# HydrogenSulfate/LFT

Measured on AMD Instinct MI355X. Metric: LF patches/sec (5x5 angRes, 32x32 LR, 4xSR), higher is better.
Workload: dtype bf16; 1 GPU; LFT 5x5 angRes 4xSR inference, batch=4 per GPU, 32x32 LR patches; global_batch=4, parallelism=dp1 (independent shards), streams_per_gpu=1, hip_graph=True, steps_in_flight=2

## Files before the change

### lft_amd/csrc/lft_api.hip

```cpp
#include "../../include/lft_hip.h"
#include "../../include/lft_hip_test.h"
#include <hip/hip_runtime.h>
#include <stdint.h>

#include <cstdarg>
#include <cstdio>
#include <cmath>
#include <map>
#include <mutex>
#include <set>
#include <string>
#include <algorithm>
#include <type_traits>
#include <utility>
#include <vector>

#ifndef LFT_TU
#define LFT_TU 0
#endif

namespace {
#include "lft_kernels_a.cuh"
#include "lft_kernels_b.cuh"
#include "lft_metrics.cuh"
// ... 92 lines not shown
    return fail(LFT_ERR_ARG, "internal: no kernel variant for %d", (int)v);
}
template <int V> using int_c = std::integral_constant<int, V>;
template <typename F> int by_prec(int prec, F&& f) {
    if (prec == LFT_PREC_F32) return f(float{});
    if (prec == LFT_PREC_BF16) return f(bf16_t{});
    return f(f16_t{});
}
inline size_t align256(size_t x) { return (x + 255) & ~(size_t)255; }

struct Dims {
    int B, A, V, h, w, hw, s, gp, gt, nchunk;
    long long ntok;
};

int make_dims(int B, int A, int h, int w, int s, int prec, Dims* d) {
    if (prec != LFT_PREC_F32 && prec != LFT_PREC_BF16 && prec != LFT_PREC_F16)
        return fail(LFT_ERR_ARG, "prec must be LFT_PREC_F32, LFT_PREC_BF16 or LFT_PREC_F16, got %d", prec);
    if (B < 1 || A < 1 || h < 1 || w < 1) return fail(LFT_ERR_SHAPE, "B, A, h, w must be positive (B=%d A=%d h=%d w=%d)", B, A, h, w);
    if (s != 2 && s != 4) return fail(LFT_ERR_SHAPE, "scale factor must be 2 or 4, got %d", s);
    if (A * A > 128) return fail(LFT_ERR_UNSUPPORTED, "angRes %d (A*A=%d views > 128) is not implemented in this build", A, A * A);
    if ((long long)B * A * A * h * w > (1LL << 27)) return fail(LFT_ERR_SHAPE, "too many tokens");
    d->B = B; d->A = A; d->V = A * A; d->h = h; d->w = w; d->hw = h * w; d->s = s;
    d->gp = (s + 2) * (s + 2); d->gt = (d->gp + 31) / 32; d->nchunk = 2 * s * s;
    d->ntok = (long long)B * d->V * d->hw;
    return 0;
}

constexpr int kFragsConv = 72, kFragsAng = 64, kFragsSpa1 = 240, kFragsSpa1NoQ = 208, kFragsSpa2 = 176;
inline int frags_up(const Dims& d) { return d.nchunk * (4 + 2 * d.gt); }

struct PackedLayout {
    size_t conv0_w, ln_ang[kLayers], ln_spa[kLayers], ang_pe, petok[kLayers], spa_pe_img;
    size_t w01, s_w01;
    size_t s_conv[3], s_ang[kLayers], s_spa1[kLayers], s_spa2[kLayers], s_up, total;
};

PackedLayout packed_layout(const Dims& d, int prec) {
    const size_t esz = prec == LFT_PREC_F32 ? 4 : 2, fragb = 64 * 8 * esz;
    PackedLayout L;
    size_t o = 0;
    auto take = [&](size_t bytes) { size_t r = o; o = align256(o + bytes); return r; };
    L.conv0_w = take(576 * 4);
    for (int l = 0; l < kLayers; ++l) { L.ln_ang[l] = take(256 * 4); L.ln_spa[l] = take(512 * 4); }
    L.ang_pe = take((size_t)((d.V + 31) / 32) * 2048 * 4);
    for (int l = 0; l < kLayers; ++l) L.petok[l] = take((size_t)((d.hw + 32 * kNwSpa1 - 1) / (32 * kNwSpa1)) * kNwSpa1 * 4096 * esz);
    L.spa_pe_img = take((size_t)d.hw * 64 * esz);
    const bool lp = prec != LFT_PREC_F32;
    L.w01 = take(lp ? 64 * kW01K * 4 : 0);
    L.s_conv[0] = take(kFragsConv * fragb);
    L.s_w01 = take(lp ? kW01Frags * fragb : 0);
    for (int i = 1; i < 3; ++i) L.s_conv[i] = take(kFragsConv * fragb);
    for (int l = 0; l < kLayers; ++l) {
        L.s_ang[l] = take(kFragsAng * fragb);
        L.s_spa1[l] = take(kFragsSpa1 * fragb);
        L.s_spa2[l] = take(kFragsSpa2 * fragb);
    }
    L.s_up = take((size_t)frags_up(d) * fragb);
    L.total = o;
    return L;
}

struct WorkLayout {
    size_t x0, feat, xa, xb, tok, q, k, v, o, g, status, total;
};
WorkLayout work_layout(const Dims& d, int prec) {
    const size_t esz = prec == LFT_PREC_F32 ? 4 : 2;
    WorkLayout W;
    size_t o = 0;
    auto take = [&](size_t bytes) { size_t r = o; o = align256(o + bytes); return r; };
    const size_t n = (size_t)d.ntok;
    W.x0 = take(n * 64 * esz); W.feat = take(n * 64 * esz); W.xa = take(n * 64 * esz); W.xb = take(n * 64 * esz);
    W.tok = take(n * 128 * esz); W.q = take(n * 128 * esz); W.k = take(n * 128 * esz); W.v = take(n * 128 * esz);
    W.o = take(n * 128 * esz);
    W.g = take(n * d.gp * 4);
    W.status = take(256);
    W.total = o;
    return W;
}

template <typename T> size_t lds_conv64(int w) { return WRing<T, kConv64Chunk, kNwConv>::LDS_BYTES + ConvIn<T, kNwConv>::bytes(w) + kNwConv * TileIO<2, T>::BYTES + kConvZeroRow; }
template <typename T> size_t lds_conv64_lr(int w) { return lds_conv64<T>(w) + std::max<size_t>(LrStage<kNwConv>::bytes(w), kConv0WBytes); }
constexpr size_t kLdsParams = 1024;
template <typename T, int CH = kSpaChunk> size_t lds_spa1(int w) {
    return WRing<T, CH, kNwSpa1>::LDS_BYTES + std::max<size_t>(ConvIn<T, kNwSpa1>::bytes(w), (size_t)kNwSpa1 * TileIO<4, T>::BYTES) + kLdsParams + kConvZeroRow;
}
template <typename T> size_t lds_spa2() { return WRing<T, kSpaChunk, kNwSpa2>::LDS_BYTES + kLdsParams + kNwSpa2 * TileIO<4, T>::BYTES; }
template <typename T> size_t lds_up() { return WRing<T, kUpChunk, kNwUp>::LDS_BYTES + kNwUp * TileIO<2, T>::BYTES; }
template <typename T> size_t lds_ang() { return (size_t)kFragsAng * 1024 * FragInfo<T>::PIECES + kLdsParams + 4 * TileIO<2, T>::BYTES; }
constexpr size_t kMaxLds = 160 * 1024;
template <typename K> int allow_lds(K kernel, size_t bytes, const char* name) {
    if (bytes > kMaxLds) return fail(LFT_ERR_SHAPE, "%s needs %zu B of LDS (> 160 KiB): view width too large for this build", name, bytes);
    if (bytes <= 64 * 1024) return 0;
    struct Done { int dev; const void* fn; size_t bytes; };
    static thread_local std::vector<Done> done;
    const void* fn = reinterpret_cast<const void*>(kernel);
    int dev = 0;
    LFT_HIP_OK(hipGetDevice(&dev));
    for (const auto& d : done)
        if (d.dev == dev && d.fn == fn && d.bytes >= bytes) return 0;
    LFT_HIP_OK(hipFuncSetAttribute(fn, hipFuncAttributeMaxDynamicSharedMemorySize, (int)bytes));
    done.push_back(Done{dev, fn, bytes});
    return 0;
}

template <typename P> P* at(const void* base, size_t off) { return reinterpret_cast<P*>(const_cast<char*>(static_cast<const char*>(base)) + off); }
inline unsigned blocks_for(long long items, int per_block) { return (unsigned)((items + per_block - 1) / per_block); }

PackOp lin_op(const float* src, int row0, int nrows, int ld, int k0, int ksteps, int kmap, float scale, int kmul = 1, int kadd = 0) {
    PackOp p{};
    p.src = src; p.kind = 0; p.row0 = row0; p.nrows = nrows; p.ntiles = (nrows + 31) / 32; p.ld = ld;
    p.kmul = kmul; p.kadd = kadd; p.k0 = k0; p.ksteps = ksteps; p.kmap = kmap; p.scale = scale; p.s = 0; p.frag0 = 0;
    return p;
}
void conv_ops(std::vector<PackOp>& v, const float* w, int nout) {
    for (int tap = 0; tap < 9; ++tap)
        for (int ks = 0; ks < 4; ++ks) v.push_back(lin_op(w, 0, nout, 576, 16 * ks, 1, 0, 1.0f, 9, tap));
}

template <typename T>
int run_pack(std::vector<PackOp>& ops, T* dst, int expect_frags, hipStream_t st) {
    int total = 0;
    size_t i = 0;
    while (i < ops.size()) {
        PackArgs a{};
        int nf = 0;
        while (i < ops.size() && a.nops < LFT_PACK_MAXOPS) {
            a.op[a.nops] = ops[i];
            a.op[a.nops].frag0 = nf;
            nf += ops[i].ntiles * ops[i].ksteps;
            ++a.nops; ++i;
        }
        k_pack<T><<<nf, 64, 0, st>>>(a, dst + (size_t)total * 512);
        LFT_LAUNCH_OK("k_pack");
        total += nf;
    }
    if (total != expect_frags) return fail(LFT_ERR_ARG, "internal: stream has %d fragments, expected %d", total, expect_frags);
    return 0;
}

template <typename T> bool tok_lane_major(const Dims& d) {
    return d.hw % (32 * kNwSpa1) == 0 && (sizeof(T) == 4 || d.w % 32 == 0);
}
template <typename T, bool PE_ONLY>
int launch_spa1(unsigned nwg, const T* in, const T* ws, const float* ln, const T* petok, T* tok, T* q, T* k, T* v, T* pe_out,
                int nimg, const Dims& d, hipStream_t st, unsigned* status) {
    const size_t l16 = lds_spa1<T, 16>(d.w), l8 = lds_spa1<T, 8>(d.w);
    const size_t share = kMaxLds / kSpaOcc;
    const bool use8 = (l16 > share && l8 <= share) || l16 > kMaxLds;
    const bool lm = !PE_ONLY && tok_lane_major<T>(d);
    return dispatch<8, 16>(use8 ? 8 : 16, [&](auto CH) {
        return dispatch<true, false>(lm, [&](auto LM) {
            constexpr bool WQ = !(LM && sizeof(T) == 2);
            const size_t lds = CH == 8 ? l8 : l16;
            if (int rc = allow_lds(k_spa1<T, PE_ONLY, CH, LM, WQ>, lds, "k_spa1")) return rc;
            k_spa1<T, PE_ONLY, CH, LM, WQ><<<nwg, 64 * kNwSpa1, lds, st>>>(in, ws, ln, petok, tok, q, k, v, pe_out, nimg, d.h, d.w, status);
            return 0;
        });
    });
}

template <typename T>
int pack_impl(const float* const* P, void* packed, const Dims& d, int prec, hipStream_t st) {
    const PackedLayout L = packed_layout(d, prec);
    const float kAngScale = 0.35355339059327373f * LFT_LOG2E;
    const float kSpaScale = 0.25f * LFT_LOG2E;
    int rc;
    k_copy_f32<<<3, 256, 0, st>>>(P[0], at<float>(packed, L.conv0_w), 576);
    LFT_LAUNCH_OK("k_copy_f32");
    for (int i = 0; i < 3; ++i) {
        std::vector<PackOp> ops;
        conv_ops(ops, P[1 + i], 64);
        if ((rc = run_pack<T>(ops, at<T>(packed, L.s_conv[i]), kFragsConv, st))) return rc;
    }
    if constexpr (sizeof(T) == 2) {
        k_compose_w01<<<blocks_for(64 * kW01K, 256), 256, 0, st>>>(P[0], P[1], at<float>(packed, L.w01));
        LFT_LAUNCH_OK("k_compose_w01");
        std::vector<PackOp> ops{lin_op(at<float>(packed, L.w01), 0, 64, kW01K, 0, kW01K / 16, 0, 1.0f)};
        if ((rc = run_pack<ConvLrOp>(ops, at<ConvLrOp>(packed, L.s_w01), kW01Frags, st))) return rc;
    }
    k_pe_tables<T><<<blocks_for(std::max<long long>((long long)((d.V + 31) / 32) * 2048, (long long)d.hw * 64), 256), 256, 0, st>>>(
        at<float>(packed, L.ang_pe), at<T>(packed, L.spa_pe_img), d.V, d.h, d.w);
    LFT_LAUNCH_OK("k_pe_tables");
    for (int l = 0; l < kLayers; ++l) {
        const float* const* q = P + 4 + 18 * l;
        float* lnS = at<float>(packed, L.ln_spa[l]);
        float* lnA = at<float>(packed, L.ln_ang[l]);
        const int srcS[4] = {1, 2, 5, 6}, srcA[4] = {10, 11, 14, 15};
        for (int j = 0; j < 4; ++j) {
            k_copy_f32<<<1, 256, 0, st>>>(q[srcS[j]], lnS + 128 * j, 128);
            k_copy_f32<<<1, 256, 0, st>>>(q[srcA[j]], lnA + 64 * j, 64);
        }
        LFT_LAUNCH_OK("k_copy_f32");
        {
            std::vector<PackOp> ops;
            ops.push_back(lin_op(q[12], 0, 64, 64, 0, 4, 1, kAngScale));
            ops.push_back(lin_op(q[12], 64, 64, 64, 0, 4, 1, 1.0f));
            ops.push_back(lin_op(q[12], 128, 64, 64, 0, 4, 1, 1.0f));
            ops.push_back(lin_op(q[13], 0, 64, 64, 0, 4, 1, 1.0f));
            ops.push_back(lin_op(q[16], 0, 128, 64, 0, 4, 1, 1.0f));
            ops.push_back(lin_op(q[17], 0, 64, 128, 0, 8, 1, 1.0f));
            if ((rc = run_pack<T>(ops, at<T>(packed, L.s_ang[l]), kFragsAng, st))) return rc;
        }
        {
            std::vector<PackOp> ops;
            conv_ops(ops, q[0], 128);
            ops.push_back(lin_op(q[3], 256, 128, 128, 0, 8, 1, 1.0f));
            ops.push_back(lin_op(q[3], 128, 128, 128, 0, 8, 1, 1.0f));
            ops.push_back(lin_op(q[3], 0, 128, 128, 0, 8, 1, kSpaScale));
            if ((rc = run_pack<T>(ops, at<T>(packed, L.s_spa1[l]), kFragsSpa1, st))) return rc;
        }
        {
            std::vector<PackOp> ops;
            ops.push_back(lin_op(q[4], 0, 128, 128, 0, 8, (sizeof(T) == 2 && tok_lane_major<T>(d)) ? 1 : 0, 1.0f));
            for (int c = 0; c < 4; ++c) {
                ops.push_back(lin_op(q[7], 64 * c, 64, 128, 0, 8, 1, 1.0f));
                ops.push_back(lin_op(q[8], 0, 128, 256, 64 * c, 4, 1, 1.0f));
            }
            ops.push_back(lin_op(q[9], 0, 64, 128, 0, 8, 1, 1.0f));
            if ((rc = run_pack<T>(ops, at<T>(packed, L.s_spa2[l]), kFragsSpa2, st))) return rc;
        }
        if ((rc = launch_spa1<T, true>((unsigned)((d.hw + 32 * kNwSpa1 - 1) / (32 * kNwSpa1)), at<T>(packed, L.spa_pe_img), at<T>(packed, L.s_spa1[l]), nullptr, nullptr,
                                       nullptr, nullptr, nullptr, nullptr, at<T>(packed, L.petok[l]), 1, d, st, nullptr))) return rc;
        LFT_LAUNCH_OK("k_spa1<pe>");
    }
    {
        std::vector<PackOp> ops;
        for (int c = 0; c < d.nchunk; ++c) {
            ops.push_back(lin_op(P[76], 32 * c, 32, 64, 0, 4, 1, 1.0f));
            PackOp m = lin_op(P[77], 0, d.gp, 0, 32 * c, 2, 1, 1.0f);
            m.kind = 1; m.s = d.s; m.ntiles = d.gt;
            ops.push_back(m);
        }
        if ((rc = run_pack<T>(ops, at<T>(packed, L.s_up), frags_up(d), st))) return rc;
    }
    return 0;
}

void launch_assemble(const float* lr, const float* g, float* out, int B, int A, int h, int w, int s, hipStream_t st, int gld = 0, unsigned* status = nullptr) {
    const dim3 tg((unsigned)((A * w + 7) / 8) * (unsigned)((A * h + 7) / 8) * (unsigned)B);
    if (!gld) gld = (s + 2) * (s + 2);
    if (s == 2) k_assemble_t<2><<<tg, 256, 0, st>>>(lr, g, out, B, A, h, w, gld, status);
    else k_assemble_t<4><<<tg, 256, 0, st>>>(lr, g, out, B, A, h, w, gld, status);
}

template <typename T>
int init_features_x0(const void* packed, const PackedLayout& L, const float* lr, T* x0, T* ta, T* tb, T* feat, const Dims& d, hipStream_t st) {
    const int nimg = d.B * d.V, nwg = nimg * ((d.hw + 32 * kNwConv - 1) / (32 * kNwConv));
    const size_t lds = lds_conv64<T>(d.w);
    int rc;
    if ((rc = allow_lds(k_conv64<T, 0>, lds, "k_conv64"))) return rc;
    if ((rc = allow_lds(k_conv64<T, 1>, lds, "k_conv64"))) return rc;
    k_conv0<T><<<dim3((unsigned)((d.hw + kConv0Tok - 1) / kConv0Tok), (unsigned)nimg), 256, 0, st>>>(lr, at<float>(packed, L.conv0_w), x0, d.B, d.A, d.h, d.w);
    LFT_LAUNCH_OK("k_conv0");
    k_conv64<T, 0><<<nwg, 64 * kNwConv, lds, st>>>(x0, ta, nullptr, at<T>(packed, L.s_conv[0]), nimg, d.h, d.w, ConvLr{});
    LFT_LAUNCH_OK("k_conv64");
    k_conv64<T, 0><<<nwg, 64 * kNwConv, lds, st>>>(ta, tb, nullptr, at<T>(packed, L.s_conv[1]), nimg, d.h, d.w, ConvLr{});
    LFT_LAUNCH_OK("k_conv64");
    k_conv64<T, 1><<<nwg, 64 * kNwConv, lds, st>>>(tb, feat, x0, at<T>(packed, L.s_conv[2]), nimg, d.h, d.w, ConvLr{});
    LFT_LAUNCH_OK("k_conv64");
    return 0;
}
template <typename T>
int init_features(const void* packed, const PackedLayout& L, const float* lr, T* x0, T* ta, T* tb, T* feat, const Dims& d, hipStream_t st) {
    if constexpr (sizeof(T) == 4) return init_features_x0<T>(packed, L, lr, x0, ta, tb, feat, d, st);
    else {
        const int nimg = d.B * d.V, nwg = nimg * ((d.hw + 32 * kNwConv - 1) / (32 * kNwConv));
        const size_t lds = lds_conv64_lr<T>(d.w);
        int rc;
        if (L.s_w01 + kW01Frags * 1024 != L.s_conv[1]) return fail(LFT_ERR_ARG, "internal: W01 fragments are not in front of conv_init.2's stream");
        if ((rc = allow_lds(k_conv64_lr<T>, lds, "k_conv64"))) return rc;
        if ((rc = allow_lds(k_conv64<T, 2>, lds, "k_conv64"))) return rc;
        k_conv64_lr<T><<<nwg, 64 * kNwConv, lds, st>>>(lr, tb, at<T>(packed, L.s_w01), d.A, nimg, d.h, d.w);
        LFT_LAUNCH_OK("k_conv64");
        k_conv64<T, 2><<<nwg, 64 * kNwConv, lds, st>>>(tb, feat, nullptr, at<T>(packed, L.s_conv[2]), nimg, d.h, d.w,
                                                      ConvLr{lr, at<float>(packed, L.conv0_w), d.A});
        LFT_LAUNCH_OK("k_conv64");
        return 0;
    }
}
template <typename T, int CT, int LL>
int ang_multi(const void* packed, const PackedLayout& L, int l, const T* in, T* out, const Dims& d, hipStream_t st, unsigned* status) {
    constexpr bool WLDS = sizeof(T) == 2;
    constexpr int NG = (sizeof(T) == 2 && CT <= 3) ? 2 : 1;
    constexpr size_t FB = 1024 * FragInfo<T>::PIECES;
    const size_t lds = (WLDS ? 64 * FB : 0) + 1024 + (size_t)NG * CT * 8 * FB + (size_t)NG * CT * TileIO<2, T>::BYTES;
    const int npix = d.B * d.hw;
    int rc;
    const unsigned grid = std::min<unsigned>(blocks_for(npix, NG), 256u * (unsigned)std::max<size_t>(1, kMaxLds / lds));
    if ((rc = allow_lds(k_ang_multi<T, CT, WLDS, NG, LL>, lds, "k_ang_multi"))) return rc;
    k_ang_multi<T, CT, WLDS, NG, LL><<<grid, 64 * CT * NG, lds, st>>>(in, out, at<T>(packed, L.s_ang[l]), at<float>(packed, L.ln_ang[l]),
                                                                     at<float>(packed, L.ang_pe), d.V, d.hw, npix, status);
    LFT_LAUNCH_OK("k_ang");
    return 0;
}
template <typename T>
int ang_block(const void* packed, const PackedLayout& L, int l, const T* in, T* out, const Dims& d, hipStream_t st, unsigned* status = nullptr) {
    auto multi = [&](auto CT, auto LL) { return ang_multi<T, CT, LL>(packed, L, l, in, out, d, st, status); };
    if (d.V > 100) return multi(int_c<4>{}, int_c<13>{});
    if (d.V > 96) return multi(int_c<4>{}, int_c<9>{});
    if (d.V > 64) return multi(int_c<3>{}, int_c<9>{});
    if (d.V == 64) return multi(int_c<2>{}, int_c<16>{});
    if (d.V > 32) return multi(int_c<2>{}, int_c<9>{});
    const int npix = d.B * d.hw;
    const size_t lds = lds_ang<T>();
    int rc;
    const unsigned grid = std::min<unsigned>(blocks_for(npix, 4), 256u * (unsigned)std::max<size_t>(1, kMaxLds / lds));
    if ((rc = allow_lds(k_ang<T, 13>, lds, "k_ang"))) return rc;
    k_ang<T, 13><<<grid, 256, lds, st>>>(in, out, at<T>(packed, L.s_ang[l]), at<float>(packed, L.ln_ang[l]),
// ... 900 lines not shown
```

### lft_amd/csrc/lft_common.cuh

```cuda
#pragma once
#include <hip/hip_runtime.h>
#include <stdint.h>
#include <utility>

typedef __bf16 bf16_t;
typedef float f32x2 __attribute__((ext_vector_type(2)));
__device__ __forceinline__ f32x2 p2_fma(f32x2 a, f32x2 b, f32x2 c) { return __builtin_elementwise_fma(a, b, c); }
typedef float f32x4 __attribute__((ext_vector_type(4)));
typedef float f32x16 __attribute__((ext_vector_type(16)));
typedef __bf16 bf16x4 __attribute__((ext_vector_type(4)));
typedef __bf16 bf16x8 __attribute__((ext_vector_type(8)));
typedef _Float16 f16_t;
typedef _Float16 f16x4 __attribute__((ext_vector_type(4)));
typedef _Float16 f16x8 __attribute__((ext_vector_type(8)));
template <typename T> struct H16;
template <> struct H16<bf16_t> { typedef bf16x4 v4; typedef bf16x8 v8; };
template <> struct H16<f16_t> { typedef f16x4 v4; typedef f16x8 v8; };
typedef unsigned int raw16 __attribute__((ext_vector_type(4), may_alias));

#define LFT_DEV static __device__ __forceinline__
#define LFT_MEM __device__ __forceinline__

#ifdef LFT_EXPERIMENT
#include "lft_experiment.cuh"
#else
#define LFT_STAMP(slot) ((void)0)
#define LFT_STAMP_IT(slot, it_ofs) ((void)0)
#endif

LFT_DEV int xcd_tile(int bid, int nwg) {
    const int q = nwg >> 3, r = nwg & 7, xcd = bid & 7;
    return (xcd < r ? xcd * (q + 1) : r * (q + 1) + (xcd - r) * q) + (bid >> 3);
}

constexpr int LFT_C = 64;
constexpr int LFT_E = 128;
constexpr float LFT_LN_EPS = 1e-5f;
constexpr float LFT_LOG2E = 1.4426950408889634f;

template <typename T> struct Frag { typename H16<T>::v8 v; };
template <> struct Frag<float> { f32x4 lo, hi; };

LFT_DEV void mma(const Frag<float>& a, const Frag<float>& b, f32x16& c) {
#pragma unroll
    for (int j = 0; j < 4; ++j) c = __builtin_amdgcn_mfma_f32_32x32x2f32(a.lo[j], b.lo[j], c, 0, 0, 0);
#pragma unroll
    for (int j = 0; j < 4; ++j) c = __builtin_amdgcn_mfma_f32_32x32x2f32(a.hi[j], b.hi[j], c, 0, 0, 0);
}
LFT_DEV f32x16 mfma16(bf16x8 a, bf16x8 b, f32x16 c) { return __builtin_amdgcn_mfma_f32_32x32x16_bf16(a, b, c, 0, 0, 0); }
LFT_DEV f32x16 mfma16(f16x8 a, f16x8 b, f32x16 c) { return __builtin_amdgcn_mfma_f32_32x32x16_f16(a, b, c, 0, 0, 0); }
template <typename T> LFT_DEV void mma(const Frag<T>& a, const Frag<T>& b, f32x16& c) { c = mfma16(a.v, b.v, c); }

LFT_DEV Frag<float> frag_zero(float) { Frag<float> f; f.lo = f32x4{0, 0, 0, 0}; f.hi = f.lo; return f; }
template <typename T> LFT_DEV Frag<T> frag_zero(T) {
    Frag<T> f;
#pragma unroll
    for (int j = 0; j < 8; ++j) f.v[j] = (T)0.0f;
    return f;
}
LFT_DEV Frag<float> frag_half(const Frag<float>& f, int which) {
    Frag<float> g = f;
    if (which == 0) g.hi = f32x4{0, 0, 0, 0}; else g.lo = f32x4{0, 0, 0, 0};
    return g;
}
template <typename T> LFT_DEV Frag<T> frag_half(const Frag<T>& f, int which) {
    Frag<T> g = f;
#pragma unroll
    for (int j = 0; j < 4; ++j) g.v[which == 0 ? j + 4 : j] = (T)0.0f;
    return g;
}
template <typename T> LFT_DEV Frag<T> frag_select(bool keep, const Frag<T>& f) { return keep ? f : frag_zero(T()); }

LFT_DEV int acc_row(int i, int h) { return (i & 3) + 8 * (i >> 2) + 4 * h; }

LFT_DEV Frag<float> acc_to_frag(const f32x16& a, int s, float) {
    Frag<float> f;
#pragma unroll
    for (int j = 0; j < 4; ++j) { f.lo[j] = a[8 * s + j]; f.hi[j] = a[8 * s + 4 + j]; }
    return f;
}
template <typename T> LFT_DEV Frag<T> acc_to_frag(const f32x16& a, int s, T) {
    Frag<T> f;
#pragma unroll
    for (int j = 0; j < 8; ++j) f.v[j] = (T)a[8 * s + j];
    return f;
}

template <typename T> struct FragInfo { static constexpr int PIECES = 1; };
template <> struct FragInfo<float> { static constexpr int PIECES = 2; };

LFT_DEV raw16 load_raw16(const char* p) { return *reinterpret_cast<const raw16*>(p); }
LFT_DEV void store_raw16(char* p, raw16 v) { *reinterpret_cast<raw16*>(p) = v; }

LFT_DEV Frag<float> frag_from_pieces(const char* base, int lane, float) {
    Frag<float> r;
    r.lo = __builtin_bit_cast(f32x4, load_raw16(base + lane * 16));
    r.hi = __builtin_bit_cast(f32x4, load_raw16(base + 1024 + lane * 16));
    return r;
}
template <typename T> LFT_DEV Frag<T> frag_from_pieces(const char* base, int lane, T) {
    Frag<T> r;
    r.v = __builtin_bit_cast(typename H16<T>::v8, load_raw16(base + lane * 16));
    return r;
}
template <typename T> LFT_DEV Frag<T> load_wfrag(const T* __restrict__ stream, int f, int lane) {
    return frag_from_pieces(reinterpret_cast<const char*>(stream) + (size_t)f * 1024 * FragInfo<T>::PIECES, lane, T());
}

LFT_DEV void glds_piece(const char* __restrict__ gsrc, char* lds_dst, int lane) {
    __builtin_amdgcn_global_load_lds((const __attribute__((address_space(1))) void*)(gsrc + lane * 16),
                                     (__attribute__((address_space(3))) void*)lds_dst, 16, 0, 0);
}

LFT_DEV void glds16_asm(const char* gsrc_lane, char* lds_dst) {
    unsigned keep;
    const unsigned dst = (unsigned)(size_t)(__attribute__((address_space(3))) char*)lds_dst;
    asm volatile("s_mov_b32 %0, m0\n\ts_mov_b32 m0, %2\n\ts_nop 0\n\tglobal_load_lds_dwordx4 %1, off\n\ts_mov_b32 m0, %0"
                 : "=&s"(keep) : "v"(gsrc_lane), "s"(dst) : "memory");
}

#define LFT_VMCNT_CASE(n) case n: asm volatile("s_waitcnt vmcnt(" #n ")" ::: "memory"); break;
LFT_DEV void wait_vmcnt(int n) {
    switch (n < 0 ? 0 : (n > 63 ? 63 : n)) {
        LFT_VMCNT_CASE(0) LFT_VMCNT_CASE(1) LFT_VMCNT_CASE(2) LFT_VMCNT_CASE(3) LFT_VMCNT_CASE(4) LFT_VMCNT_CASE(5) LFT_VMCNT_CASE(6) LFT_VMCNT_CASE(7)
        LFT_VMCNT_CASE(8) LFT_VMCNT_CASE(9) LFT_VMCNT_CASE(10) LFT_VMCNT_CASE(11) LFT_VMCNT_CASE(12) LFT_VMCNT_CASE(13) LFT_VMCNT_CASE(14) LFT_VMCNT_CASE(15)
        LFT_VMCNT_CASE(16) LFT_VMCNT_CASE(17) LFT_VMCNT_CASE(18) LFT_VMCNT_CASE(19) LFT_VMCNT_CASE(20) LFT_VMCNT_CASE(21) LFT_VMCNT_CASE(22) LFT_VMCNT_CASE(23)
        LFT_VMCNT_CASE(24) LFT_VMCNT_CASE(25) LFT_VMCNT_CASE(26) LFT_VMCNT_CASE(27) LFT_VMCNT_CASE(28) LFT_VMCNT_CASE(29) LFT_VMCNT_CASE(30) LFT_VMCNT_CASE(31)
        LFT_VMCNT_CASE(32) LFT_VMCNT_CASE(33) LFT_VMCNT_CASE(34) LFT_VMCNT_CASE(35) LFT_VMCNT_CASE(36) LFT_VMCNT_CASE(37) LFT_VMCNT_CASE(38) LFT_VMCNT_CASE(39)
        LFT_VMCNT_CASE(40) LFT_VMCNT_CASE(41) LFT_VMCNT_CASE(42) LFT_VMCNT_CASE(43) LFT_VMCNT_CASE(44) LFT_VMCNT_CASE(45) LFT_VMCNT_CASE(46) LFT_VMCNT_CASE(47)
        LFT_VMCNT_CASE(48) LFT_VMCNT_CASE(49) LFT_VMCNT_CASE(50) LFT_VMCNT_CASE(51) LFT_VMCNT_CASE(52) LFT_VMCNT_CASE(53) LFT_VMCNT_CASE(54) LFT_VMCNT_CASE(55)
        LFT_VMCNT_CASE(56) LFT_VMCNT_CASE(57) LFT_VMCNT_CASE(58) LFT_VMCNT_CASE(59) LFT_VMCNT_CASE(60) LFT_VMCNT_CASE(61) LFT_VMCNT_CASE(62) LFT_VMCNT_CASE(63)
    }
}

LFT_DEV void wg_barrier_keep_vm() { asm volatile("s_waitcnt lgkmcnt(0)\n\ts_barrier" ::: "memory"); }
LFT_DEV void wg_barrier_keep_vm_lds_visible() {
    __builtin_amdgcn_s_waitcnt(0xC07F);
    asm volatile("s_barrier" ::: "memory");
}

#define LFT_NOTE_ASM_(kind, ring, slot) asm volatile("; LFT_NOTE " kind " ring=%0 slot=%1" :: "i"(ring), "i"(slot))
#define LFT_DMA_NOTE(kind, ring, slot) do { if (__builtin_constant_p(slot)) LFT_NOTE_ASM_(kind, ring, slot); } while (0)
constexpr int kNoteWRing = 0, kNoteWRingPipe = 1, kNoteKV = 2, kNoteConvIn = 3, kNoteAngW = 4;

template <typename T, int CH, int NW = 4>
struct WRing {
    static constexpr int NBUF = 3;
    static constexpr int FRAG_BYTES = 1024 * FragInfo<T>::PIECES;
    static constexpr int CHUNK_BYTES = CH * FRAG_BYTES;
    static constexpr int LDS_BYTES = NBUF * CHUNK_BYTES;
    static constexpr int PIECES_PER_WAVE = CH * FragInfo<T>::PIECES / NW;
    static_assert((CH * FragInfo<T>::PIECES) % NW == 0, "chunk must split over the workgroup's waves");
    static_assert(PIECES_PER_WAVE <= 12, "counted vmcnt immediates below cover up to 12 pieces per wave");
    const char* g;
    char* lds;
    int lane, wave, pos, nfrag;
    LFT_MEM void init(const T* stream, char* lds_base, int total_frags) {
        g = reinterpret_cast<const char*>(stream); lds = lds_base; nfrag = total_frags; pos = 0;
        lane = threadIdx.x & 63;
        wave = __builtin_amdgcn_readfirstlane(threadIdx.x >> 6);
        issue(0);
        issue(1);
    }
    LFT_MEM void issue(int c) {
        if (c * CH >= nfrag) return;
        const char* src = g + (size_t)c * CHUNK_BYTES;
        char* dst = lds + (c % NBUF) * CHUNK_BYTES;
        const int last = (nfrag - c * CH) * FragInfo<T>::PIECES - 1;
        LFT_DMA_NOTE("DMA", kNoteWRing, c % NBUF);
#pragma unroll
        for (int i = 0; i < PIECES_PER_WAVE; ++i) {
            const int piece = min(wave * PIECES_PER_WAVE + i, last);
            glds_piece(src + piece * 1024, dst + piece * 1024, lane);
        }
    }
    LFT_MEM void wait_landed(bool next_in_flight) { wait_vmcnt(next_in_flight ? PIECES_PER_WAVE : 0); }
    LFT_MEM Frag<T> next() {
        const int c = pos / CH, i = pos % CH;
        if (i == 0) {
            if (c > 0) LFT_DMA_NOTE("DONE", kNoteWRing, (c + NBUF - 1) % NBUF);
            wait_landed((c + 1) * CH < nfrag);
            wg_barrier_keep_vm();
            issue(c + 2);
            LFT_DMA_NOTE("USE", kNoteWRing, c % NBUF);
        }
        ++pos;
        return frag_from_pieces(lds + (c % NBUF) * CHUNK_BYTES + i * FRAG_BYTES, lane, T());
    }
};


template <typename T, int CH, int NW, int NBUF, int NFRAG>
struct WRingPipe {
    static constexpr int FRAG_BYTES = 1024 * FragInfo<T>::PIECES;
    static constexpr int CHUNK_BYTES = CH * FRAG_BYTES;
    static constexpr int LDS_BYTES = NBUF * CHUNK_BYTES;
    static constexpr int PIECES_PER_WAVE = CH * FragInfo<T>::PIECES / NW;
    static constexpr int NCHUNK = (NFRAG + CH - 1) / CH;
    static_assert((CH * FragInfo<T>::PIECES) % NW == 0, "chunk must split over the workgroup's waves");
    static_assert(PIECES_PER_WAVE * (NBUF - 1) <= 63, "counted vmcnt immediate");
    static constexpr int cmin(int a, int b) { return a < b ? a : b; }
    static constexpr int cmax(int a, int b) { return a > b ? a : b; }
    const char* g;
    char* lds;
    int lane, wave, split_slot, split_gap;
    Frag<T> fr0[CH], fr1[CH];
    LFT_MEM void setup(const T* stream, char* lds_base, int split_slot_ = NBUF, int split_gap_ = 0) {
        g = reinterpret_cast<const char*>(stream); lds = lds_base;
        split_slot = split_slot_; split_gap = split_gap_;
        lane = threadIdx.x & 63;
        wave = __builtin_amdgcn_readfirstlane(threadIdx.x >> 6);
    }
    LFT_MEM char* slot(int c) const {
        const int s = c % NBUF;
        return lds + s * CHUNK_BYTES + (s >= split_slot ? split_gap : 0);
    }
    LFT_MEM void issue(int c) {
        if (c * CH >= NFRAG) return;
        const char* src = g + (size_t)c * CHUNK_BYTES;
        char* dst = slot(c);
        const int last = (NFRAG - c * CH) * FragInfo<T>::PIECES - 1;
        LFT_DMA_NOTE("DMA", kNoteWRingPipe, c % NBUF);
#pragma unroll
        for (int i = 0; i < PIECES_PER_WAVE; ++i) {
            const int piece = min(wave * PIECES_PER_WAVE + i, last);
            glds_piece(src + piece * 1024, dst + piece * 1024, lane);
        }
    }
    template <int C> LFT_MEM void fetch() {
        const char* base = slot(C);
        LFT_NOTE_ASM_("USE", kNoteWRingPipe, C % NBUF);
#pragma unroll
        for (int i = 0; i < CH; ++i)
            if (C * CH + i < NFRAG) {
                if constexpr (C & 1) fr1[i] = frag_from_pieces(base + i * FRAG_BYTES, lane, T());
                else fr0[i] = frag_from_pieces(base + i * FRAG_BYTES, lane, T());
            }
        LFT_NOTE_ASM_("DONE", kNoteWRingPipe, C % NBUF);
    }
    LFT_MEM void init(const T* stream, char* lds_base) {
        setup(stream, lds_base);
#pragma unroll
        for (int c = 0; c < NBUF; ++c) issue(c);
    }
    LFT_MEM void start() {
        wait_vmcnt(cmax(0, cmin(NBUF - 1, NCHUNK - 1)) * PIECES_PER_WAVE);
        wg_barrier_keep_vm_lds_visible();
        fetch<0>();
        __builtin_amdgcn_sched_barrier(0);
    }
    template <int POS> LFT_MEM Frag<T> get() {
        constexpr int C = POS / CH, I = POS % CH;
        static_assert(POS >= 0 && POS < NFRAG, "position outside the stream");
        if constexpr (I == 0 && C + 1 < NCHUNK) {
            __builtin_amdgcn_sched_barrier(0);
            wait_vmcnt(cmax(0, cmin(NBUF - 2, NCHUNK - 2 - C)) * PIECES_PER_WAVE);
            wg_barrier_keep_vm_lds_visible();
            issue(C + NBUF);
            fetch<C + 1>();
            __builtin_amdgcn_sched_barrier(0);
        }
        if constexpr (C & 1) return fr1[I];
        else return fr0[I];
    }
};
template <int POS0, int NT_OUT, int KS, typename Ring, typename T, int... I>
LFT_DEV void linear_ring_seq(Ring& ring, const Frag<T> (&x)[KS], f32x16 (&y)[NT_OUT], std::integer_sequence<int, I...>) {
    (mma(ring.template get<POS0 + I>(), x[I % KS], y[I / KS]), ...);
}
template <int POS0, int NT_OUT, int KS, typename Ring, typename T>
LFT_DEV void linear_ring_at(Ring& ring, const Frag<T> (&x)[KS], f32x16 (&y)[NT_OUT]) {
    linear_ring_seq<POS0, NT_OUT, KS>(ring, x, y, std::make_integer_sequence<int, NT_OUT * KS>());
}
LFT_DEV Frag<float> load_row8(const float* __restrict__ p, bool ok, float) {
    Frag<float> r;
    const f32x4* q = reinterpret_cast<const f32x4*>(p);
    r.lo = q[0]; r.hi = q[1];
    if (!ok) r = frag_zero(0.0f);
    return r;
}
template <typename T> LFT_DEV Frag<T> load_row8(const T* __restrict__ p, bool ok, T) {
    Frag<T> r;
    r.v = *reinterpret_cast<const typename H16<T>::v8*>(p);
    if (!ok) r = frag_zero(T());
    return r;
}

LFT_DEV Frag<float> lds_row8(const char* p, bool ok, float) {
    Frag<float> r;
    r.lo = __builtin_bit_cast(f32x4, load_raw16(p));
    r.hi = __builtin_bit_cast(f32x4, load_raw16(p + 16));
    if (!ok) r = frag_zero(0.0f);
    return r;
}
template <typename T> LFT_DEV Frag<T> lds_row8(const char* p, bool ok, T) {
    Frag<T> r;
    r.v = __builtin_bit_cast(typename H16<T>::v8, load_raw16(p));
    if (!ok) r = frag_zero(T());
    return r;
}

LFT_DEV f32x4 load4(const float* p) { return *reinterpret_cast<const f32x4*>(p); }
template <typename T> LFT_DEV f32x4 load4(const T* p) {
    typename H16<T>::v4 v = *reinterpret_cast<const typename H16<T>::v4*>(p);
    return f32x4{(float)v[0], (float)v[1], (float)v[2], (float)v[3]};
}
LFT_DEV void store4(float* p, f32x4 v) { *reinterpret_cast<f32x4*>(p) = v; }
template <typename T> LFT_DEV void store4(T* p, f32x4 v) {
    typename H16<T>::v4 o;
#pragma unroll
    for (int j = 0; j < 4; ++j) o[j] = (T)v[j];
    *reinterpret_cast<typename H16<T>::v4*>(p) = o;
}

template <int NT, typename T>
LFT_DEV void load_acc(const T* __restrict__ row, bool ok, int h, f32x16 (&a)[NT]) {
#pragma unroll
    for (int nt = 0; nt < NT; ++nt) {
#pragma unroll
        for (int g = 0; g < 4; ++g) {
            const f32x4 v = load4(row + 32 * nt + 8 * g + 4 * h);
#pragma unroll
            for (int j = 0; j < 4; ++j) a[nt][4 * g + j] = ok ? v[j] : 0.0f;
        }
    }
}
template <typename T> struct RawPiece { typedef typename H16<T>::v4 type; };
template <> struct RawPiece<float> { typedef f32x4 type; };
template <int NT, typename T>
// ... 321 lines not shown
LFT_DEV float opaque_inf() { float v; asm("s_mov_b32 %0, 0x7f800000" : "=s"(v)); return v; }
LFT_DEV float relu_fast(float x) { return __builtin_amdgcn_fmed3f(x, 0.0f, opaque_inf()); }
LFT_DEV float lrelu02_fast(float x) { return __builtin_amdgcn_fmed3f(x, 0.2f * x, opaque_inf()); }
LFT_DEV float max_fast(float a, float b) { return __builtin_amdgcn_fmed3f(a, b, opaque_inf()); }
LFT_DEV void xhalf_split(float v, float& lo, float& hi) {
    lo = v; hi = v;
    asm volatile("s_nop 1\n\tv_permlane32_swap_b32 %0, %1" : "+v"(lo), "+v"(hi));
}
LFT_DEV float xhalf_sum(float v) { float lo, hi; xhalf_split(v, lo, hi); return lo + hi; }
LFT_DEV float xhalf_max(float v) { float lo, hi; xhalf_split(v, lo, hi); return max_fast(lo, hi); }

typedef unsigned int u32x2 __attribute__((ext_vector_type(2)));
typedef short s16x4v __attribute__((ext_vector_type(4)));
LFT_DEV f32x4 mfma16k16(u32x2 a, u32x2 b, f32x4 c, bf16_t) {
    return __builtin_amdgcn_mfma_f32_16x16x16bf16_1k(__builtin_bit_cast(s16x4v, a), __builtin_bit_cast(s16x4v, b), c, 0, 0, 0);
}
LFT_DEV f32x4 mfma16k16(u32x2 a, u32x2 b, f32x4 c, f16_t) {
    return __builtin_amdgcn_mfma_f32_16x16x16f16(__builtin_bit_cast(f16x4, a), __builtin_bit_cast(f16x4, b), c, 0, 0, 0);
}
LFT_DEV f32x4 mfma16k32(bf16x8 a, bf16x8 b, f32x4 c) { return __builtin_amdgcn_mfma_f32_16x16x32_bf16(a, b, c, 0, 0, 0); }
LFT_DEV f32x4 mfma16k32(f16x8 a, f16x8 b, f32x4 c) { return __builtin_amdgcn_mfma_f32_16x16x32_f16(a, b, c, 0, 0, 0); }
LFT_DEV void swap16(unsigned& d, unsigned& s) { asm volatile("s_nop 1\n\tv_permlane16_swap_b32 %0, %1" : "+v"(d), "+v"(s)); }
LFT_DEV void swap16(float& d, float& s) { asm volatile("s_nop 1\n\tv_permlane16_swap_b32 %0, %1" : "+v"(d), "+v"(s)); }
LFT_DEV void swap32(float& d, float& s) { asm volatile("s_nop 1\n\tv_permlane32_swap_b32 %0, %1" : "+v"(d), "+v"(s)); }
LFT_DEV void frag_to_blocks(raw16& f) {
    unsigned a0 = f[0], a1 = f[1], b0 = f[2], b1 = f[3];
    swap16(a0, b0);
    swap16(a1, b1);
    f = raw16{a0, a1, b0, b1};
}
template <typename OP> LFT_DEV void xrow_combine2(float& a, float& b, OP op) {
    swap16(a, b);
    float c = op(a, b), c2 = c;
    swap32(c, c2);
    float d = op(c, c2), d2 = d;
    swap16(d, d2);
    a = d; b = d2;
}

LFT_DEV float fast_rcp(float x) { return __builtin_amdgcn_rcpf(x); }
LFT_DEV unsigned not_finite(float v) { return !(__builtin_fabsf(v) < 3.0e38f); }
template <int NT, bool FAST = false>
LFT_DEV void layernorm_acc(f32x16 (&a)[NT], const float* gamma, const float* beta, int h, unsigned& bad) {
    if constexpr (FAST) {
        f32x2 s2 = {0.0f, 0.0f};
#pragma unroll
        for (int nt = 0; nt < NT; ++nt)
#pragma unroll
            for (int i = 0; i < 16; i += 2) s2 += f32x2{a[nt][i], a[nt][i + 1]};
        const float mean = xhalf_sum(s2[0] + s2[1]) * (1.0f / (NT * 32));
        const f32x2 mean2 = {mean, mean};
        f32x2 q2 = {0.0f, 0.0f};
#pragma unroll
        for (int nt = 0; nt < NT; ++nt)
#pragma unroll
            for (int i = 0; i < 16; i += 2) {
                const f32x2 d = f32x2{a[nt][i], a[nt][i + 1]} - mean2;
                q2 = p2_fma(d, d, q2);
                a[nt][i] = d[0]; a[nt][i + 1] = d[1];
            }
        const float var = xhalf_sum(q2[0] + q2[1]) * (1.0f / (NT * 32)) + LFT_LN_EPS;
        bad |= not_finite(var);
        const float rstd = __builtin_amdgcn_rsqf(var);
        const f32x2 rstd2 = {rstd, rstd};
#pragma unroll
        for (int nt = 0; nt < NT; ++nt)
#pragma unroll
            for (int g = 0; g < 4; ++g) {
                const f32x4 gm = __builtin_bit_cast(f32x4, load_raw16(reinterpret_cast<const char*>(gamma + 32 * nt + 8 * g + 4 * h)));
                const f32x4 bt = __builtin_bit_cast(f32x4, load_raw16(reinterpret_cast<const char*>(beta + 32 * nt + 8 * g + 4 * h)));
#pragma unroll
                for (int j = 0; j < 4; j += 2) {
                    const f32x2 sc = f32x2{gm[j], gm[j + 1]} * rstd2;
                    const f32x2 o = p2_fma(f32x2{a[nt][4 * g + j], a[nt][4 * g + j + 1]}, sc, f32x2{bt[j], bt[j + 1]});
                    a[nt][4 * g + j] = o[0]; a[nt][4 * g + j + 1] = o[1];
                }
            }
        return;
    }
    float s = 0.0f;
#pragma unroll
    for (int nt = 0; nt < NT; ++nt)
#pragma unroll
        for (int i = 0; i < 16; ++i) s += a[nt][i];
    const float mean = xhalf_sum(s) * (1.0f / (NT * 32));
    float q = 0.0f;
#pragma unroll
    for (int nt = 0; nt < NT; ++nt)
#pragma unroll
        for (int i = 0; i < 16; ++i) { float d = a[nt][i] - mean; q += d * d; }
    const float var = xhalf_sum(q) * (1.0f / (NT * 32)) + LFT_LN_EPS;
    bad |= not_finite(var);
    const float rstd = FAST ? __builtin_amdgcn_rsqf(var) : 1.0f / sqrtf(var);
#pragma unroll
    for (int nt = 0; nt < NT; ++nt)
#pragma unroll
        for (int g = 0; g < 4; ++g) {
            const f32x4 gm = __builtin_bit_cast(f32x4, load_raw16(reinterpret_cast<const char*>(gamma + 32 * nt + 8 * g + 4 * h)));
            const f32x4 bt = __builtin_bit_cast(f32x4, load_raw16(reinterpret_cast<const char*>(beta + 32 * nt + 8 * g + 4 * h)));
#pragma unroll
            for (int j = 0; j < 4; ++j) a[nt][4 * g + j] = (a[nt][4 * g + j] - mean) * rstd * gm[j] + bt[j];
        }
}
constexpr unsigned LFT_STATUS_NONFINITE_BIT = 1u;
LFT_DEV void publish_status(unsigned* status, unsigned bad) {
    if (bad && status) *status = LFT_STATUS_NONFINITE_BIT;
}
LFT_DEV raw16 params_load(const float* __restrict__ src, int n) {
    const int i = min((int)threadIdx.x * 4, n - 4);
    return load_raw16(reinterpret_cast<const char*>(src + i));
}
LFT_DEV void params_store(float* lds_dst, int n, raw16 v) {
    const int i = threadIdx.x * 4;
    if (i < n) store_raw16(reinterpret_cast<char*>(lds_dst + i), v);
}

template <int NT, typename T>
LFT_DEV void acc_frags(const f32x16 (&a)[NT], Frag<T> (&f)[2 * NT]) {
#pragma unroll
    for (int nt = 0; nt < NT; ++nt) {
        f[2 * nt] = acc_to_frag(a[nt], 0, T());
        f[2 * nt + 1] = acc_to_frag(a[nt], 1, T());
    }
}

template <int NT>
LFT_DEV void acc_frags_relu(const f32x16 (&a)[NT], Frag<float> (&f)[2 * NT]) {
#pragma unroll
    for (int nt = 0; nt < NT; ++nt)
#pragma unroll
        for (int s = 0; s < 2; ++s) {
#pragma unroll
            for (int j = 0; j < 4; ++j) { f[2 * nt + s].lo[j] = relu_fast(a[nt][8 * s + j]); f[2 * nt + s].hi[j] = relu_fast(a[nt][8 * s + 4 + j]); }
        }
}
template <int NT, typename T>
LFT_DEV void acc_frags_relu(const f32x16 (&a)[NT], Frag<T> (&f)[2 * NT]) {
    typedef short s16x8 __attribute__((ext_vector_type(8)));
    acc_frags<NT, T>(a, f);
#pragma unroll
    for (int k = 0; k < 2 * NT; ++k) {
        const s16x8 v = __builtin_bit_cast(s16x8, f[k].v);
        f[k].v = __builtin_bit_cast(typename H16<T>::v8, __builtin_elementwise_max(v, (s16x8)(0)));
    }
}

template <int NT_OUT, int KS, typename T, int CH, int NW>
LFT_DEV void linear_ring(WRing<T, CH, NW>& ring, const Frag<T> (&x)[KS], f32x16 (&y)[NT_OUT]) {
#pragma unroll
    for (int nt = 0; nt < NT_OUT; ++nt)
#pragma unroll
        for (int ks = 0; ks < KS; ++ks) mma(ring.next(), x[ks], y[nt]);
}

template <int NT_OUT, int KS, typename T>
LFT_DEV void linear_acc(const T* __restrict__ w, int f0, int lane, const Frag<T> (&x)[KS], f32x16 (&y)[NT_OUT]) {
#pragma unroll
    for (int nt = 0; nt < NT_OUT; ++nt)
#pragma unroll
        for (int ks = 0; ks < KS; ++ks) mma(load_wfrag(w, f0 + nt * KS + ks, lane), x[ks], y[nt]);
}
```

### lft_amd/csrc/lft_kernels_b.cuh

```cuda
#pragma once
#include "lft_common.cuh"
#include "lft_kernels_a.cuh"

constexpr int kUpChunk = 8;
constexpr int kSpaChunk = 16;
constexpr int kSpaOcc = 2;
constexpr int kNwSpa1 = 4, kNwSpa2 = 4, kNwUp = 8;
template <typename T, bool PE_ONLY, int CH = kSpaChunk, bool TOKLM = false, bool WITH_Q = true, int NW = kNwSpa1>
__global__ __launch_bounds__(64 * NW, kSpaOcc) void k_spa1(const T* __restrict__ X, const T* __restrict__ ws,
                                              const float* __restrict__ ln, const T* __restrict__ petok,
                                              T* __restrict__ TOK, T* __restrict__ Q, T* __restrict__ K, T* __restrict__ Vv,
                                              T* __restrict__ pe_out, int nimg, int h, int w, unsigned* __restrict__ status) {
    extern __shared__ __attribute__((aligned(16))) char smem[];
    const int lane = threadIdx.x & 63, r = lane & 31, hh = lane >> 5, wave = threadIdx.x >> 6;
    constexpr int TT = 32 * NW;
    const int hw = h * w, tpi = (hw + TT - 1) / TT;
    const int bid = xcd_tile(blockIdx.x, gridDim.x);
    const int im = bid / tpi, p0 = (bid % tpi) * TT;
    const int tl = wave * 32 + r, p = p0 + tl;
    const bool ok = p < hw;
    LFT_STAMP(0);
    typename RawPiece<T>::type pe_raw[16];
    if (!PE_ONLY) load_lane_major_raw<4, T>(petok + (size_t)((p0 >> 5) + wave) * 4096, lane, pe_raw);
    char* lds_in = smem + WRing<T, CH, NW>::LDS_BYTES;
    float* lds_ln = reinterpret_cast<float*>(lds_in + max(ConvIn<T, NW>::bytes(w), NW * TileIO<4, T>::BYTES));
    char* zero_row = reinterpret_cast<char*>(lds_ln) + 1024;
    raw16 lnv = raw16{0u, 0u, 0u, 0u};
    if (!PE_ONLY) lnv = params_load(ln, 256);
    WRing<T, CH, NW> ring;
    ring.init(ws, smem, PE_ONLY ? 144 : (WITH_Q ? 240 : 208));
    stage_conv_input<T, NW>(X + (size_t)im * hw * 64, p0, hw, w, lds_in);
    clear_zero_row(zero_row);
    LFT_STAMP(12);
    wait_staged();
    LFT_STAMP(13);
    if (!PE_ONLY) params_store(lds_ln, 256, lnv);
    __syncthreads();
    LFT_NOTE_ASM_("USE", kNoteConvIn, 0);
    LFT_STAMP(1);
    f32x16 t[4];
    zero_acc<4>(t);
    conv3x3_tile<4, T, NW>(lds_in, zero_row, tl, p / w, p % w, ok, h, w, hh, ring, t);
    LFT_STAMP(2);
    if (PE_ONLY) {
        store_lane_major<4, T>(pe_out + (size_t)((p0 >> 5) + wave) * 4096, lane, t);
        return;
    }
    __syncthreads();
    LFT_STAMP(3);
    const int t0 = p0 + wave * 32, nvalid = max(0, min(32, hw - t0));
    const size_t tile_off = ((size_t)im * hw + min(t0, hw - 1)) * 128;
    char* scr = lds_in + wave * TileIO<4, T>::BYTES;
    if constexpr (TOKLM) store_tile_lm<4, T>(TOK + ((size_t)im * hw + t0) * 128, lane, t);
    else store_tile<4, T>(TOK + tile_off, nvalid, lane, t, scr);
    LFT_STAMP(4);
    Frag<T> nf[8];
    constexpr bool QKVLM = TOKLM && sizeof(T) == 2;
    const size_t lm_off = ((size_t)im * hw + t0) * 128;
    acc_frags<4, T>(t, nf);
#pragma unroll
    for (int half = 0; half < 2; ++half) {
        f32x16 a[2];
        zero_acc<2>(a);
        linear_ring<2, 8, T>(ring, nf, a);
        if constexpr (QKVLM) store_tile_lm<2, T>(Vv + lm_off + half * 2048, lane, a);
        else store_tile<2, T, 128>(Vv + tile_off + 64 * half, nvalid, lane, a, scr);
    }
    LFT_STAMP(6);
    add_acc_raw<4, T>(t, pe_raw, ok);
    unsigned bad = 0;
    layernorm_acc<4, sizeof(T) == 2>(t, lds_ln, lds_ln + 128, hh, bad);
    acc_frags<4, T>(t, nf);
    LFT_STAMP(7);
#pragma unroll
    for (int half = 0; half < 2; ++half) {
        f32x16 a[2];
        zero_acc<2>(a);
        linear_ring<2, 8, T>(ring, nf, a);
        if constexpr (QKVLM) store_tile_lm<2, T>(K + lm_off + half * 2048, lane, a);
        else store_tile<2, T, 128>(K + tile_off + 64 * half, nvalid, lane, a, scr);
    }
    LFT_STAMP(9);
    if constexpr (WITH_Q) {
#pragma unroll
        for (int half = 0; half < 2; ++half) {
            f32x16 a[2];
            zero_acc<2>(a);
            linear_ring<2, 8, T>(ring, nf, a);
            if constexpr (QKVLM) store_tile_lm<2, T>(Q + lm_off + half * 2048, lane, a);
            else store_tile<2, T, 128>(Q + tile_off + 64 * half, nvalid, lane, a, scr);
        }
    }
    LFT_STAMP(11);
    publish_status(status, bad);
}

constexpr int kAttTY = 4, kAttTX = 32, kAttHR = kAttTY + 4, kAttHC = kAttTX + 4;
LFT_DEV int att_swz(int row, int col) { return (row & 1) | (((col >> 2) & 1) << 1); }
typedef short s16x4 __attribute__((ext_vector_type(4)));

template <typename T, bool SKIP, bool TOKLM = false, bool YLM = false, int NW = kNwSpa2>
__global__ __launch_bounds__(64 * NW, kSpaOcc) void k_spa2(const T* __restrict__ TOK, const T* __restrict__ O, const T* __restrict__ ws,
                                              const float* __restrict__ ln, const T* __restrict__ skip, T* __restrict__ Y,
                                              long long ntok, unsigned* __restrict__ status) {
    extern __shared__ __attribute__((aligned(16))) char smem[];
    const int lane = threadIdx.x & 63, r = lane & 31, hh = lane >> 5;
    const int wave = threadIdx.x >> 6;
    const long long t0 = ((long long)blockIdx.x * NW + wave) * 32;
    const int nvalid = (int)max(0LL, min(32LL, ntok - t0));
    const long long tb = min(t0, ntok - 1);
    char* scr = smem + WRing<T, kSpaChunk, NW>::LDS_BYTES + 1024 + wave * TileIO<4, T>::BYTES;
    WRing<T, kSpaChunk, NW> ring;
    LFT_STAMP(16);
    ring.init(ws, smem, 176);
    f32x16 t[4], n[4];
    if constexpr (TOKLM) load_tile_lm<4, T>(TOK + tb * 128, lane, t);
    else load_tile<4, T>(TOK + tb * 128, nvalid, lane, t, scr);
    Frag<T> f[8];
    load_tile_frags<8, T>(O + tb * 128, nvalid, lane, f, scr);
    f32x16 sk[2];
    if (SKIP) load_tile<2, T>(skip + tb * 64, nvalid, lane, sk, scr);
    float* lds_ln = reinterpret_cast<float*>(smem + WRing<T, kSpaChunk, NW>::LDS_BYTES);
    params_store(lds_ln, 256, params_load(ln + 256, 256));
    LFT_STAMP(17);
    linear_ring<4, 8, T>(ring, f, t);
    LFT_STAMP(18);
#pragma unroll
    for (int nt = 0; nt < 4; ++nt) n[nt] = t[nt];
    unsigned bad = 0;
    layernorm_acc<4>(n, lds_ln, lds_ln + 128, hh, bad);
    acc_frags<4, T>(n, f);
    LFT_STAMP(19);
#pragma unroll
    for (int c = 0; c < 4; ++c) {
        f32x16 hid[2];
        zero_acc<2>(hid);
        linear_ring<2, 8, T>(ring, f, hid);
        Frag<T> hf[4];
        acc_frags_relu<2>(hid, hf);
        linear_ring<4, 4, T>(ring, hf, t);
    }
    LFT_STAMP(20);
    acc_frags<4, T>(t, f);
    f32x16 y[2];
    zero_acc<2>(y);
    linear_ring<2, 8, T>(ring, f, y);
    if (SKIP) {
#pragma unroll
        for (int nt = 0; nt < 2; ++nt) y[nt] += sk[nt];
    }
    LFT_STAMP(21);
    if constexpr (YLM) store_tile_lm<2, T>(Y + tb * 64, lane, y);
    else store_tile<2, T>(Y + tb * 64, nvalid, lane, y, scr);
    LFT_STAMP(22);
    publish_status(status, bad);
}

constexpr int kSpaBChunk = 8;
constexpr int kAdTile = kAttHR * kAttHC * 64;
constexpr int kAdPerWave = 2 * kAdTile / 1024 / 4;
static_assert(2 * kAdTile == 4 * kAdPerWave * 1024, "the K and V tiles must split into whole pieces over 4 waves");
constexpr int kSpaBLds = 4 * kAdTile + 2048;
constexpr int kSpaBSlotsA = (2 * kAdTile) / (kSpaBChunk * 1024);
constexpr int kSpaBSlotsB = 2;
constexpr int kSpaBSlots = kSpaBSlotsA + kSpaBSlotsB;
constexpr int kSpaBScratchOfs = 16384;
static_assert(kSpaBScratchOfs + 4 * TileIO<4, bf16_t>::BYTES <= 2 * kAdTile, "scratch must fit buffer B");
static_assert(kSpaBSlotsB * kSpaBChunk * 1024 <= kSpaBScratchOfs, "the ring slots in buffer B must end before the scratch");

template <typename T> LFT_DEV void q_load_async(const T* p0, const T* p1, raw16& a, raw16& b) {
    asm volatile("global_load_dwordx4 %0, %2, off\n\tglobal_load_dwordx4 %1, %3, off" : "=&v"(a), "=&v"(b) : "v"(p0), "v"(p1) : "memory");
}
LFT_DEV void ld16_async(const void* p, raw16& d) { asm volatile("global_load_dwordx4 %0, %1, off" : "=v"(d) : "v"(p) : "memory"); }
template <int OFS> LFT_DEV void ld16_async_ofs(const void* p, raw16& d) {
    static_assert(OFS >= 0 && OFS < 4096, "global_load immediate offset");
    asm volatile("global_load_dwordx4 %0, %1, off offset:%2" : "=v"(d) : "v"(p), "n"(OFS) : "memory");
}
LFT_DEV void ld16_async_x8(const char* p, raw16 (&d)[8]) {
    const char* p2 = p + 4096;
    ld16_async_ofs<0>(p, d[0]); ld16_async_ofs<1024>(p, d[1]); ld16_async_ofs<2048>(p, d[2]); ld16_async_ofs<3072>(p, d[3]);
    ld16_async_ofs<0>(p2, d[4]); ld16_async_ofs<1024>(p2, d[5]); ld16_async_ofs<2048>(p2, d[6]); ld16_async_ofs<3072>(p2, d[7]);
}
template <int N> LFT_DEV void wait_vm_8(raw16 (&r)[8]) {
    asm volatile("s_waitcnt vmcnt(%8)" : "+v"(r[0]), "+v"(r[1]), "+v"(r[2]), "+v"(r[3]), "+v"(r[4]), "+v"(r[5]), "+v"(r[6]), "+v"(r[7]) : "n"(N) : "memory");
    __builtin_amdgcn_sched_barrier(0);
}
template <int N> LFT_DEV void wait_vm_only() {
    asm volatile("s_waitcnt vmcnt(%0)" :: "n"(N) : "memory");
    __builtin_amdgcn_sched_barrier(0);
}
template <int N> LFT_DEV void wait_vm_q(raw16& a, raw16& b) {
    asm volatile("s_waitcnt vmcnt(%2)" : "+v"(a), "+v"(b) : "n"(N) : "memory");
    __builtin_amdgcn_sched_barrier(0);
}

template <typename T> LFT_DEV void q_head_pair(const raw16 (&wr)[8], const Frag<T> (&nf)[8], Frag<T>& q0, Frag<T>& q1) {
    f32x16 q;
#pragma unroll
    for (int i = 0; i < 16; ++i) q[i] = 0.0f;
#pragma unroll
    for (int ks = 0; ks < 8; ++ks) {
        Frag<T> wf;
// ... 563 lines not shown
```

Measured before the change: 10190 patches/s.

## Keep k_spa1 V/K projection weights resident in LDS instead of streaming through ring

For the 16-bit lane-major, no-Q variant of k_spa1, the ring now streams only the conv chunks. The V projection weights are read directly from the ring slots they already occupy, and the K projection weights are prefetched into the freed ring slot and conv-input region while the V projection and layernorm run. This removes per-chunk barriers and ring waits in the projection phase and overlaps the K-weight fetch with compute. In exchange it adds a host-side shape check that fails if the LDS regions are too small, and it drains vmcnt fully before the projection phase.

```diff
diff --git a/lft_amd/csrc/lft_api.hip b/lft_amd/csrc/lft_api.hip
--- a/lft_amd/csrc/lft_api.hip
+++ b/lft_amd/csrc/lft_api.hip
@@ -268,9 +268,12 @@
     return dispatch<8, 16>(use8 ? 8 : 16, [&](auto CH) {
         return dispatch<true, false>(lm, [&](auto LM) {
             constexpr bool WQ = !(LM && sizeof(T) == 2);
+            constexpr bool RES = !PE_ONLY && !WQ && CH == 16;
+            if (RES && 3 * CH + ConvIn<T, kNwSpa1>::dma_pieces(d.w) < 64)
+                return fail(LFT_ERR_SHAPE, "internal: k_spa1's resident projection weights need 64 KiB, ring + input tile have %d", 3 * CH + ConvIn<T, kNwSpa1>::dma_pieces(d.w));
             const size_t lds = CH == 8 ? l8 : l16;
-            if (int rc = allow_lds(k_spa1<T, PE_ONLY, CH, LM, WQ>, lds, "k_spa1")) return rc;
-            k_spa1<T, PE_ONLY, CH, LM, WQ><<<nwg, 64 * kNwSpa1, lds, st>>>(in, ws, ln, petok, tok, q, k, v, pe_out, nimg, d.h, d.w, status);
+            if (int rc = allow_lds(k_spa1<T, PE_ONLY, CH, LM, WQ, RES>, lds, "k_spa1")) return rc;
+            k_spa1<T, PE_ONLY, CH, LM, WQ, RES><<<nwg, 64 * kNwSpa1, lds, st>>>(in, ws, ln, petok, tok, q, k, v, pe_out, nimg, d.h, d.w, status);
             return 0;
         });
     });
diff --git a/lft_amd/csrc/lft_common.cuh b/lft_amd/csrc/lft_common.cuh
--- a/lft_amd/csrc/lft_common.cuh
+++ b/lft_amd/csrc/lft_common.cuh
@@ -142,6 +142,7 @@
 #define LFT_NOTE_ASM_(kind, ring, slot) asm volatile("; LFT_NOTE " kind " ring=%0 slot=%1" :: "i"(ring), "i"(slot))
 #define LFT_DMA_NOTE(kind, ring, slot) do { if (__builtin_constant_p(slot)) LFT_NOTE_ASM_(kind, ring, slot); } while (0)
 constexpr int kNoteWRing = 0, kNoteWRingPipe = 1, kNoteKV = 2, kNoteConvIn = 3, kNoteAngW = 4;
+constexpr int kNoteSpa1Wk = 5;
 
 template <typename T, int CH, int NW = 4>
 struct WRing {
@@ -175,6 +176,16 @@
         }
     }
     LFT_MEM void wait_landed(bool next_in_flight) { wait_vmcnt(next_in_flight ? PIECES_PER_WAVE : 0); }
+    LFT_MEM void fetch_resident(int c, char* dst) {
+        const char* src = g + (size_t)c * CHUNK_BYTES;
+#pragma unroll
+        for (int i = 0; i < PIECES_PER_WAVE; ++i) {
+            const int piece = wave * PIECES_PER_WAVE + i;
+            glds16_asm(src + piece * 1024 + lane * 16, dst + piece * 1024);
+        }
+    }
+    LFT_MEM char* slot_base(int s) const { return lds + s * CHUNK_BYTES; }
+    LFT_MEM Frag<T> frag_at(const char* chunk, int i) const { return frag_from_pieces(chunk + i * FRAG_BYTES, lane, T()); }
     LFT_MEM Frag<T> next() {
         const int c = pos / CH, i = pos % CH;
         if (i == 0) {
@@ -802,6 +813,14 @@
 #pragma unroll
         for (int ks = 0; ks < KS; ++ks) mma(ring.next(), x[ks], y[nt]);
 }
+template <int NT_OUT, int KS, typename T, int CH, int NW>
+LFT_DEV void linear_resident(const WRing<T, CH, NW>& ring, const char* chunk, const Frag<T> (&x)[KS], f32x16 (&y)[NT_OUT]) {
+    static_assert(NT_OUT * KS == CH, "one chunk per call");
+#pragma unroll
+    for (int nt = 0; nt < NT_OUT; ++nt)
+#pragma unroll
+        for (int ks = 0; ks < KS; ++ks) mma(ring.frag_at(chunk, nt * KS + ks), x[ks], y[nt]);
+}
 
 template <int NT_OUT, int KS, typename T>
 LFT_DEV void linear_acc(const T* __restrict__ w, int f0, int lane, const Frag<T> (&x)[KS], f32x16 (&y)[NT_OUT]) {
diff --git a/lft_amd/csrc/lft_kernels_b.cuh b/lft_amd/csrc/lft_kernels_b.cuh
--- a/lft_amd/csrc/lft_kernels_b.cuh
+++ b/lft_amd/csrc/lft_kernels_b.cuh
@@ -6,7 +6,7 @@
 constexpr int kSpaChunk = 16;
 constexpr int kSpaOcc = 2;
 constexpr int kNwSpa1 = 4, kNwSpa2 = 4, kNwUp = 8;
-template <typename T, bool PE_ONLY, int CH = kSpaChunk, bool TOKLM = false, bool WITH_Q = true, int NW = kNwSpa1>
+template <typename T, bool PE_ONLY, int CH = kSpaChunk, bool TOKLM = false, bool WITH_Q = true, bool RES = false, int NW = kNwSpa1>
 __global__ __launch_bounds__(64 * NW, kSpaOcc) void k_spa1(const T* __restrict__ X, const T* __restrict__ ws,
                                               const float* __restrict__ ln, const T* __restrict__ petok,
                                               T* __restrict__ TOK, T* __restrict__ Q, T* __restrict__ K, T* __restrict__ Vv,
@@ -28,7 +28,8 @@
     raw16 lnv = raw16{0u, 0u, 0u, 0u};
     if (!PE_ONLY) lnv = params_load(ln, 256);
     WRing<T, CH, NW> ring;
-    ring.init(ws, smem, PE_ONLY ? 144 : (WITH_Q ? 240 : 208));
+    static_assert(!RES || (TOKLM && sizeof(T) == 2 && !WITH_Q && !PE_ONLY && CH == 16), "resident projection phase: 16-bit lane-major hand-off with 16-fragment chunks");
+    ring.init(ws, smem, PE_ONLY ? 144 : (WITH_Q ? 240 : (RES ? 176 : 208)));
     stage_conv_input<T, NW>(X + (size_t)im * hw * 64, p0, hw, w, lds_in);
     clear_zero_row(zero_row);
     LFT_STAMP(12);
@@ -46,8 +47,55 @@
         store_lane_major<4, T>(pe_out + (size_t)((p0 >> 5) + wave) * 4096, lane, t);
         return;
     }
+    if constexpr (RES) {
+        LFT_NOTE_ASM_("DONE", kNoteWRing, 2);
+        LFT_NOTE_ASM_("DONE", kNoteConvIn, 0);
+        asm volatile("s_waitcnt vmcnt(0)" ::: "memory");
+    }
     __syncthreads();
     LFT_STAMP(3);
+    if constexpr (RES) {
+        char* const wk0 = ring.slot_base(2);
+        LFT_NOTE_ASM_("DMA", kNoteSpa1Wk, 0);
+        ring.fetch_resident(11, wk0);
+        LFT_NOTE_ASM_("DMA", kNoteSpa1Wk, 1);
+        ring.fetch_resident(12, lds_in);
+        const size_t lm_off = ((size_t)im * hw + p0 + wave * 32) * 128;
+        store_tile_lm<4, T>(TOK + lm_off, lane, t);
+        LFT_STAMP(4);
+        Frag<T> nf[8];
+        acc_frags<4, T>(t, nf);
+#pragma unroll
+        for (int half = 0; half < 2; ++half) {
+            f32x16 a[2];
+            zero_acc<2>(a);
+            LFT_NOTE_ASM_("USE", kNoteWRing, half);
+            linear_resident<2, 8, T>(ring, ring.slot_base(half), nf, a);
+            LFT_NOTE_ASM_("DONE", kNoteWRing, half);
+            store_tile_lm<2, T>(Vv + lm_off + half * 2048, lane, a);
+        }
+        LFT_STAMP(6);
+        add_acc_raw<4, T>(t, pe_raw, ok);
+        unsigned bad = 0;
+        layernorm_acc<4, true>(t, lds_ln, lds_ln + 128, hh, bad);
+        acc_frags<4, T>(t, nf);
+        LFT_STAMP(7);
+        asm volatile("s_waitcnt vmcnt(0)" ::: "memory");
+        wg_barrier_keep_vm();
+#pragma unroll
+        for (int half = 0; half < 2; ++half) {
+            f32x16 a[2];
+            zero_acc<2>(a);
+            LFT_NOTE_ASM_("USE", kNoteSpa1Wk, half);
+            linear_resident<2, 8, T>(ring, half == 0 ? wk0 : lds_in, nf, a);
+            LFT_NOTE_ASM_("DONE", kNoteSpa1Wk, half);
+            store_tile_lm<2, T>(K + lm_off + half * 2048, lane, a);
+        }
+        LFT_STAMP(9);
+        LFT_STAMP(11);
+        publish_status(status, bad);
+        return;
+    }
     const int t0 = p0 + wave * 32, nvalid = max(0, min(32, hw - t0));
     const size_t tile_off = ((size_t)im * hw + min(t0, hw - 1)) * 128;
     char* scr = lds_in + wave * TileIO<4, T>::BYTES;
```

Result: no change. 10250 patches/s (median of 5 runs) (+0.6%).
